# sine2pi/ASR-model

Measured on AMD Instinct MI355X. Metric: audio-sec/sec fwd+bwd on 30s@16kHz LibriSpeech-shaped clips (whole job, all GPUs), higher is better.
Workload: dtype bf16; 1 GPU; tiny (BASELINE configs[1]): log-mel + 4 enc/4 dec d=384 h=6 fwd+bwd, 32 x 30 s clips per GPU, T=256; model=tiny, global_batch=32, seq_len=3001, text_len=256, pitch_frames=3001, parallelism=dp1

## Files before the change

### asr-model_amd/asrx/lib.py

```python
from __future__ import annotations

import ctypes
import os

import torch

_HERE = os.path.dirname(os.path.abspath(__file__))
LIB_PATH = os.environ.get("ASRX_LIB") or os.path.join(_HERE, "libasrx.so")

_i64 = ctypes.c_int64
_i32 = ctypes.c_int
_f32 = ctypes.c_float
_p = ctypes.c_void_p
_u32 = ctypes.c_uint32

SIGNATURES = {
    "asrx_last_error": (ctypes.c_char_p, []),
    "asrx_abi_version": (_i32, []),
    "asrx_noise_hash": (_u32, [_u32, _u32]),
    "asrx_set_noise_epoch": (_i32, [_u32, _p]),
    "asrx_set_gemm_variant": (_i32, [_i32]),
    "asrx_set_attn_variant": (_i32, [_i32]),
    "asrx_set_wgrad_variant": (_i32, [_i32]),
    "asrx_mel_frames": (_i32, [_i64]),
    "asrx_logmel_ws_bytes": (_i64, [_i64, _i64]),
    "asrx_flac_info": (_i32, [_p, _i64, _p, _p, _p, _p, _p]),
    "asrx_flac_decode": (_i32, [_p, _i64, _p, _i64]),
    "asrx_pcm_normalize": (_i32, [_p, _i32, _i64, _i64, _i64, _p, _p, _p, _i64, _i32, _p]),
    "asrx_logmel": (_i32, [_p, _i64, _i64, _i64, _p, _p, _p, _p, _i32, _i64, _p, _p, _i64, _p]),
    "asrx_gemm": (
        _i32,
        [_i32, _p, _i64, _i64, _i32, _i32, _p, _i64, _i64, _i32, _i32, _p, _i64, _i64, _p, _p,
         _i64, _i64, _i64, _i64, _f32, _f32, _i32, _i64, _i64, _i32, _p],
    ),
    "asrx_abby_fwd": (_i32, [_p, _p, _p, _p, _p, _p, _p, _i64, _i64, _i64, _i64, _i64, _u32, _i32, _p]),
    "asrx_abby_fwd_logits": (_i32, [_p, _p, _p, _p, _p, _p, _i64, _i64, _i64, _i64, _i64, _u32, _i32, _p]),
    "asrx_abby_bwd": (_i32, [_p, _p, _p, _p, _p, _p, _p, _p, _p, _p, _i64, _i64, _p]),
    "asrx_attn_fwd": (_i32, [_i32, _p, _p, _p, _p, _p, _p, _p, _p, _p, _i64, _i64, _i64, _i64, _i64, _i32, _f32, _p]),
    "asrx_attn_bwd": (_i32, [_i32, _p, _p, _p, _p, _p, _p, _p, _p, _p, _p, _p, _p, _p, _p, _p, _p, _p, _p,
                             _i64, _i64, _i64, _i64, _i64, _i32, _f32, _p]),
    "asrx_layernorm_fwd": (_i32, [_p, _p, _p, _p, _p, _p, _i64, _i64, _f32, _p]),
    "asrx_layernorm_bwd": (_i32, [_p, _p, _p, _p, _p, _p, _p, _p, _i64, _i64, _p]),
    "asrx_layernorm_bwd_acc": (_i32, [_p, _p, _p, _p, _p, _p, _p, _p, _i64, _i64, _i32, _p]),
    "asrx_small_linear_fwd": (_i32, [_p, _p, _p, _p, _i64, _i64, _i64, _i32, _p]),
    "asrx_small_linear_bwd": (_i32, [_p, _p, _p, _p, _p, _p, _p, _i64, _i64, _i64, _i32, _f32, _p]),
    "asrx_rownorm": (_i32, [_p, _p, _i64, _i64, _p]),
    "asrx_rownorm_bwd": (_i32, [_p, _p, _p, _p, _i64, _i64, _p]),
    "asrx_row_normalize": (_i32, [_p, _p, _p, _i64, _i64, _p]),
    "asrx_row_normalize_bwd": (_i32, [_p, _p, _p, _p, _i64, _i64, _i32, _p]),
    "asrx_softmax_small": (_i32, [_p, _p, _i64, _i64, _p]),
    "asrx_softmax_small_bwd": (_i32, [_p, _p, _p, _i64, _i64, _p]),
    "asrx_zero": (_i32, [_p, _i64, _p]),
    "asrx_rotary_fwd": (_i32, [_p, _p, _p, _p, _i64, _i64, _i64, _i64, _f32, _p]),
    "asrx_rotary_bwd": (_i32, [_p, _p, _p, _p, _p, _p, _i64, _i64, _i64, _i64, _f32, _p]),
    "asrx_abby_bwd2": (_i32, [_p] * 10 + [_i64, _i64, _i32, _p]),
    "asrx_rownorm_bwd2": (_i32, [_p, _p, _p, _p, _i64, _i64, _i32, _p]),
    "asrx_colsum_ld": (_i32, [_p, _i64, _p, _i64, _i64, _p]),
    "asrx_ce_fwd1": (_i32, [_p] * 6 + [_i64, _i64, _p]),
    "asrx_ce_bwd2": (_i32, [_p] * 6 + [_i64, _i64, _p]),
    "asrx_bn_running": (_i32, [_p] * 5 + [_i64, _i64, _i64, _f32, _f32, _p]),
    "asrx_rsqrt_eps": (_i32, [_p, _p, _i64, _f32, _p]),
    "asrx_conv3_weight": (_i32, [_p, _p, _i64, _i64] + [_p] * 6),
    "asrx_conv3_weight_bwd": (_i32, [_p] * 4 + [_i64, _i64] + [_p] * 3),
    "asrx_blend_fwd": (_i32, [_p] * 4 + [_i64, _p]),
    "asrx_blend_bwd": (_i32, [_p] * 7 + [_i64, _p]),
    "asrx_add_segments": (_i32, [_p, _i64, _p, _p, _p, _i64, _p]),
    "asrx_cat3": (_i32, [_p] * 3 + [_i64, _p, _p]),
    "asrx_layernorm_fwd2": (_i32, [_p] * 10 + [_i32, _i64, _i64, _f32, _p]),
    "asrx_vgate_weights": (_i32, [_p] * 7 + [_i64, _i64, _i64, _p]),
    "asrx_msheath_row_fwd": (_i32, [_p] * 6 + [_i64] + [_p] * 14 + [_i64] * 4 + [_f32, _f32, _p, _i64, _i64, _p]),
    "asrx_msheath_row_bwd": (_i32, [_p] * 11 + [_i64] + [_p] * 18 + [_i64] * 4 + [_f32, _p, _i64, _i64, _p]),
    "asrx_msheath_row_bwd2": (_i32, [_i32, _p, _p, _p, _f32, _p] + [_p] * 11 + [_i64] + [_p] * 18 + [_i64] * 4
                              + [_f32, _p, _i64, _i64, _p]),
    "asrx_gemm_wn_rows": (_i32, [_p, _i64, _p, _i64, _p, _i64, _p, _p, _i64, _i64, _i64, _f32, _f32, _i32, _i32, _p,
                                 _p, _p]),
    "asrx_row_tiles_max": (_i64, [_i64]),
    "asrx_wgrad_bf16": (_i32, [_p, _i64, _p, _i64, _p, _i64, _i64, _i64, _i64, _i64, _p]),
    "asrx_pitch_dio": (_i32, [_p, _i64, _i64, _i64] + [ctypes.c_double] * 5 + [_p, _i64, _p, _p, _p, _p, _i64]
                       + [_p] * 4 + [_i64] + [_p] * 4 + [_i64, _p]),
    "asrx_pitch_stonemask": (_i32, [_p, _i64, _i64, _i64, ctypes.c_double, _p, ctypes.c_double, _i64, _p, _p]),
    "asrx_wconv_entry_bytes": (_i64, []),
    "asrx_weights_to_bf16": (_i32, [_p, _i64, _i64, _p]),
    "asrx_row_tiles": (_i32, [_p, _i64, _i64, _i64, _p, _p, _p]),
    "asrx_msheath_ctrl_fwd3": (_i32, [_p, _p, _i64, _p, _p, _p, _p, _p, _i64, _p, _p, _p, _p] + [_i64] * 5 + [_p] * 8),
    "asrx_mem_chunks": (_i64, [_i64]),
    "asrx_seg_colsum_det": (_i32, [_p, _p, _p, _i64, _i64, _i64, _f32, _p]),
    "asrx_msheath_ctrl_bwd3": (_i32, [_p, _p, _p, _p, _p, _p, _i64, _p, _p, _p] + [_i64] * 4 + [_p, _i32] + [_p] * 8),
    "asrx_axpy_row2_colsum": (_i32, [_p] * 6 + [_i64] * 3 + [_p, _i64, _p]),
    "asrx_vgate_fwd": (_i32, [_p, _p, _p, _p, _p, _p, _p, _p, _p, _p, _p, _p, _p, _i64, _i64, _i64, _f32, _p]),
    "asrx_vgate_bwd": (_i32, [_p, _p, _p, _p, _p, _p, _p, _p, _p, _p, _p, _p, _p, _p, _p, _p, _p,
                              _i64, _i64, _i64, _f32, _p]),
    "asrx_tgate_fwd": (_i32, [_p, _p, _p, _i64, _i64, _p]),
    "asrx_tgate_bwd": (_i32, [_p, _p, _p, _p, _p, _i64, _i64, _p]),
    "asrx_axpy_row": (_i32, [_p, _p, _p, _p, _i64, _i64, _p]),
    "asrx_axpy_row_bwd": (_i32, [_p, _p, _p, _p, _p, _i64, _i64, _p]),
    "asrx_axpy_row_bwd2": (_i32, [_p, _p, _p, _p, _p, _p, _i64, _i64, _p]),
    "asrx_jump_select": (_i32, [_p, _p, _p, _p, _p, _p, _p, _p, _i64, _i64, _i64, _p]),
    "asrx_jump_select_bwd": (_i32, [_p, _p, _p, _p, _p, _p, _p, _p, _p, _p, _p, _p, _i64, _i64, _i64, _p]),
    "asrx_seg_colsum": (_i32, [_p, _p, _i64, _i64, _i64, _f32, _i32, _p]),
    "asrx_msheath_ctrl_fwd": (_i32, [_p, _p, _i64, _p, _p, _p, _p, _p, _p, _i64, _i64, _i64, _i64, _i64,
                                     _p, _p, _p, _p, _p, _p, _p, _p]),
    "asrx_msheath_ctrl_bwd": (_i32, [_p, _p, _p, _p, _p, _p, _p, _p, _p, _i64, _i64, _i64, _i64, _p, _p, _p, _p, _p,
                                     _p]),
    "asrx_msheath_rec_bytes": (_i64, []),
    "asrx_msheath_ctrl_fwd2": (_i32, [_p, _p, _i64, _p, _p, _p, _i64, _p, _p, _p, _i64, _i64, _i64, _i64, _i64,
                                      _p, _p, _p, _p, _p, _p, _p, _p]),
    "asrx_msheath_ctrl_bwd2": (_i32, [_p, _p, _p, _p, _p, _p, _i64, _p, _p, _p, _i64, _i64, _i64, _i64, _p, _i32,
                                      _p, _p, _p, _p, _p, _p]),
    "asrx_jump_select4_bwd_acc": (_i32, [_p, _p, _p, _p, _p, _p, _p, _p, _p, _p, _p, _p, _p, _i64, _i64, _i64, _p]),
    "asrx_jump_bwd_part_floats": (_i64, [_i64, _i64, _i64]),
    "asrx_jump_select4_bwd_part": (_i32, [_p] * 11 + [_i64, _i64, _i64, _p]),
    "asrx_msheath_ctrl_bwd4": (_i32, [_p, _i64, _p, _p, _p, _i64, _p, _p, _p, _i64, _i64, _i64, _i64, _p, _i32]
                               + [_p] * 8),
    "asrx_axpy_row2_bwd_acc": (_i32, [_p, _p, _f32, _p, _p, _p, _p, _p, _p, _p, _p, _i64, _i64, _i64, _p]),
    "asrx_jump_select4_bwd_part2": (_i32, [_p] * 11 + [_i64, _i64, _i64, _p]),
    "asrx_jump_select4_bwd_acc2": (_i32, [_p] * 13 + [_i64, _i64, _i64, _p]),
    "asrx_axpy_row2_bwd_acc2": (_i32, [_p, _p, _p, _f32, _p, _p, _p, _p, _p, _p, _p, _p, _i64, _i64, _i64, _p]),
    "asrx_wgrad_split": (_i32, [_p, _i64, _p, _i32, _i64, _p, _i64, _p, _i64, _i64, _i64, _i64, _i64, _i64, _p]),
    "asrx_msheath_dx_final": (_i32, [_p, _p, _p, _p, _i64, _i64, _i64, _p]),
    "asrx_axpy_row2": (_i32, [_p, _p, _p, _p, _p, _i64, _i64, _p]),
    "asrx_axpy_row2_bwd": (_i32, [_p, _p, _p, _p, _p, _p, _p, _i64, _i64, _p]),
    "asrx_jump_select4": (_i32, [_p, _p, _p, _p, _p, _p, _p, _p, _i64, _i64, _i64, _p]),
    "asrx_jump_select4_bwd": (_i32, [_p, _p, _p, _p, _p, _p, _p, _p, _p, _p, _p, _p, _i64, _i64, _i64, _p]),
    "asrx_colsum": (_i32, [_p, _p, _i64, _i64, _p]),
    "asrx_add_rows": (_i32, [_p, _p, _p, _p, _i64, _i64, _i64, _p]),
    "asrx_lincomb": (_i32, [_p, _p, _p, _f32, _f32, _f32, _p, _i64, _p]),
    "asrx_act_fwd": (_i32, [_p, _p, _i64, _i32, _p]),
    "asrx_act_bwd": (_i32, [_p, _p, _p, _i64, _i32, _p]),
    "asrx_glu_fwd": (_i32, [_p, _p, _i64, _i64, _p]),
    "asrx_glu_bwd": (_i32, [_p, _p, _p, _i64, _i64, _p]),
    "asrx_dropout": (_i32, [_p, _p, _i64, _i64, _i64, _i64, _u32, _f32, _p]),
    "asrx_act_dropout_fwd": (_i32, [_p, _p, _p, _i64, _i64, _i64, _i64, _u32, _f32, _i32, _i32, _p]),
    "asrx_act_dropout_bwd": (_i32, [_p, _p, _p, _i64, _i64, _i64, _i64, _u32, _f32, _i32, _i32, _p]),
    "asrx_dwconv_fwd": (_i32, [_p, _p, _p, _p, _i64, _i64, _i64, _i64, _p]),
    "asrx_dwconv_bwd": (_i32, [_p, _p, _p, _p, _p, _p, _i64, _i64, _i64, _i64, _p]),
    "asrx_bn_fwd": (_i32, [_p, _p, _p, _p, _p, _p, _i64, _i64, _i64, _f32, _i32, _p]),
    "asrx_bn_bwd": (_i32, [_p, _p, _p, _p, _p, _p, _p, _p, _p, _p, _i64, _i64, _i64, _p]),
    "asrx_dwconv_pre_bwd": (_i32, [_p, _p, _p, _p, _p, _p, _p, _i64, _i64, _i64, _i64, _i32, _p]),
    "asrx_bn_silu_fwd": (_i32, [_p, _p, _p, _p, _p, _p, _i64, _i64, _i64, _f32, _i32, _p]),
    "asrx_bn_silu_bwd": (_i32, [_p, _p, _p, _p, _p, _p, _p, _p, _p, _p, _p, _i64, _i64, _i64, _p]),
    "asrx_stem1_fwd": (_i32, [_p, _p, _p, _p, _i64, _i64, _i64, _p]),
    "asrx_stem1_bwd": (_i32, [_p, _p, _p, _p, _i64, _i64, _i64, _p]),
    "asrx_embed_fwd": (_i32, [_p, _p, _p, _i64, _i64, _p]),
    "asrx_embed_bwd": (_i32, [_p, _p, _p, _i64, _i64, _p]),
    "asrx_ce_fwd": (_i32, [_p, _p, _p, _p, _i64, _i64, _p]),
    "asrx_ce_bwd": (_i32, [_p, _p, _p, _p, _p, _i64, _i64, _p]),
    "asrx_policy_noise": (_i32, [_p, _i64, _i64, _i64, _u32, _p]),
    "asrx_weight_to_bf16": (_i32, [_p, _p, _i64, _i64, _i64, _i32, _p]),
    "asrx_gemm_wn_router": (_i32, [_p, _i64, _p, _i64, _p, _p, _p, _i64, _p, _i64, _i64, _i64, _p]),
    "asrx_gemm_wn": (_i32, [_p, _i64, _i32, _i64, _i64, _p, _i64, _p, _i64, _p, _p, _i64, _i64, _i64, _f32, _f32,
                            _i32, _i32, _p]),
    "asrx_gemm_wn_ex": (_i32, [_p, _i32, _i64, _i32, _i64, _i64, _p, _i64, _p, _i32, _i64, _p, _p, _i64, _i64, _i64,
                               _f32, _f32, _i32, _i32, _p, _p, _p]),
    "asrx_wgrad_bf16_ex": (_i32, [_p, _i64, _p, _i32, _i64, _p, _i64, _i64, _i64, _i64, _i64, _p]),
    "asrx_abby_fwd2": (_i32, [_p, _p, _p, _p, _p, _i32, _p, _p, _i64, _i64, _i64, _i64, _i64, _u32, _i32, _p, _p, _p,
                              _p]),
    "asrx_gemm_wn_gact": (_i32, [_p, _i32, _i64, _p, _i64, _p, _p, _i64, _p, _i64, _p, _i64, _i64, _i64, _i32, _i32,
                                 _p]),
    "asrx_rotary_table": (_i32, [_p, _p, _i64, _i64, _p]),
    "asrx_rotary_fwd2": (_i32, [_p, _p, _p, _p, _p, _i64, _i64, _i64, _i64, _f32, _p]),
    "asrx_rotary_bwd2": (_i32, [_p, _p, _p, _p, _p, _p, _p, _i64, _i64, _i64, _i64, _f32, _p]),
    "asrx_abby_fwd3": (_i32, [_p, _p, _p, _p, _p, _p, _i32, _p, _p, _i64, _i64, _i64, _i64, _i64, _u32, _i32, _p, _p,
                               _p, _p, _p]),
    "asrx_abby_fwd_logits2": (_i32, [_p, _p, _p, _p, _i32, _p, _p, _i64, _i64, _i64, _i64, _i64, _u32, _i32, _p, _p,
                                     _p, _p]),
    "asrx_attn_fwd2": (_i32, [_i32, _i32, _p, _p, _p, _p, _p, _p, _p, _p, _p, _i64, _i64, _i64, _i64, _i64, _i32, _f32,
                              _p]),
    "asrx_attn_bwd2": (_i32, [_i32, _i32, _p, _p, _p, _p, _p, _p, _p, _p, _p, _p, _p, _p, _p, _p, _p, _p, _p, _p,
                              _i64, _i64, _i64, _i64, _i64, _i32, _f32, _p]),
    "asrx_small_linear_fwd2": (_i32, [_p, _i32, _p, _p, _p, _i64, _i64, _i64, _i32, _p]),
    "asrx_small_linear_bwd2": (_i32, [_p, _p, _p, _i32, _p, _p, _p, _p, _i64, _i64, _i64, _i32, _f32, _p]),
    "asrx_tgate_fwd2": (_i32, [_p, _p, _p, _i32, _i64, _i64, _p]),
    "asrx_msheath_row_fwd2": (_i32, [_p] * 6 + [_i64] + [_p] * 7 + [_i32] + [_p] * 7 + [_i64] * 4
                                    + [_f32, _f32, _p, _i64, _i64, _p]),
    "asrx_msheath_row_fwd3": (_i32, [_p] * 6 + [_i64] + [_p] * 16 + [_i64] * 4 + [_f32, _f32, _p, _i64, _i64, _p]),
# ... 125 lines not shown
```

### asr-model_amd/csrc/attn_mf.hip

```cpp
#include "common.h"

namespace asrx {

struct AttnStridesMF {
  int64_t b, l, h;
};

typedef short v4i16 __attribute__((ext_vector_type(4)));
typedef __attribute__((address_space(3))) v4i16 lds_v4i16;

namespace amf {

constexpr int QB = 256;
constexpr int KT = 64;
constexpr int NTHR = 512;
constexpr int HALF = KT * 64;
constexpr float LOG2E = 1.4426950408889634f;
constexpr float LN2 = 0.6931471805599453f;

__device__ __forceinline__ int kswz(int key) { return (key >> 1) & 7; }
__device__ __forceinline__ int vswz(int key) { return ((key >> 1) & 1) << 2; }

__device__ __forceinline__ unsigned pack2(float a, float b) {
  typedef __attribute__((ext_vector_type(2))) float f2;
// ... 546 lines not shown
          const int ql = 32 * qb2 + 8 * (2 * s2 + e4) + 4 * hi;
          const float4 lo = *reinterpret_cast<const float4*>(&LD[buf][ql]);
          const float4 hi4 = *reinterpret_cast<const float4*>(&LD[buf][ql + 2]);
          const float l2v[4] = {lo.x, lo.z, hi4.x, hi4.z}, dlv[4] = {lo.y, lo.w, hi4.y, hi4.w};
#pragma unroll
          for (int e = 0; e < 4; e += 2) {
            typedef __attribute__((ext_vector_type(2))) float f2;
            const int r = 8 * s2 + 4 * e4 + e;
            const f2 a = __builtin_elementwise_fma((f2){sacc[r], sacc[r + 1]}, (f2){c, c}, (f2){-l2v[e], -l2v[e + 1]});
            f2 p = {__builtin_amdgcn_exp2f(a.x), __builtin_amdgcn_exp2f(a.y)};
            if (need_mask) {
              p.x = kq > ql + e ? 0.f : p.x;
              p.y = kq > ql + e + 1 ? 0.f : p.y;
            }
            const f2 ds = p * ((f2){pacc[r], pacc[r + 1]} - (f2){dlv[e], dlv[e + 1]});
            pv[4 * e4 + e] = p.x;
            pv[4 * e4 + e + 1] = p.y;
            dsv[4 * e4 + e] = ds.x;
            dsv[4 * e4 + e + 1] = ds.y;
          }
        }
        const bf16x8 pb = pack8(pv), sb = pack8(dsv);
#pragma unroll
        for (int d = 0; d < HD / 32; ++d) {
          dvacc[d] = __builtin_amdgcn_mfma_f32_32x32x16_bf16(tr_frag(Dt[buf] + (d >> 1) * HALF, lane, qb2, s2, d & 1),
                                                             pb, dvacc[d], 0, 0, 0);
          dkacc[d] = __builtin_amdgcn_mfma_f32_32x32x16_bf16(tr_frag(Qt[buf] + (d >> 1) * HALF, lane, qb2, s2, d & 1),
                                                             sb, dkacc[d], 0, 0, 0);
        }
      }
    }
    if (t + 1 < ntiles) stage_st(buf ^ 1);
    __syncthreads();
  }

  if (key < Lk) {
    store_rowT<HD>(dk + b * sdk.b + h * sdk.h + key * sdk.l, dkacc, scale, hi);
    store_rowT<HD>(dv + b * sdv.b + h * sdv.h + key * sdv.l, dvacc, 1.f, hi);
  }
}

template <int HD, typename TI = float, typename TD = float>
__global__ __launch_bounds__(BwdCfg<HD>::NT, 1) void attn_bwd_dq_mf_kernel(
    const TI* __restrict__ q, const TI* __restrict__ k, const TI* __restrict__ v,
    const TD* __restrict__ dO, const float* __restrict__ lse, const float* __restrict__ delta,
    float* __restrict__ dq, AttnStridesMF sq, AttnStridesMF sk, AttnStridesMF sv, AttnStridesMF sd,
    AttnStridesMF sdq, int64_t H, int64_t Lq, int64_t Lk, int causal, float scale) {
  typedef BwdCfg<HD> C;
  constexpr int NH = HD / 64;
  __shared__ __attribute__((aligned(16))) unsigned short Kr[2][NH * HALF], Kt2[2][NH * HALF], Vr[2][NH * HALF];

  const int64_t nqb = (Lq + 32 * C::NW - 1) / (32 * C::NW), L = xcd_logical(blockIdx.x, gridDim.x);
  const int b = (int)(L / (nqb * H)), h = (int)((L / nqb) % H);
  const int64_t q0 = (L % nqb) * (32 * C::NW);
  const int tid = threadIdx.x, lane = tid & 63, wid = __builtin_amdgcn_readfirstlane(tid >> 6);
  const int j = lane & 31, hi = lane >> 5;
  const int64_t qi = q0 + wid * 32 + j;
  const TI* kbp = k + b * sk.b + h * sk.h;
  const TI* vbp = v + b * sv.b + h * sv.h;
  const float c = scale * LOG2E;

  bf16x8 qf[HD / 16], gf[HD / 16];
  row_frags<HD>(q + b * sq.b + h * sq.h, sq.l, qi, Lq, hi, qf);
  row_frags<HD>(dO + b * sd.b + h * sd.h, sd.l, qi, Lq, hi, gf);
  const float l2 = qi < Lq ? lse[((int64_t)b * H + h) * Lq + qi] * LOG2E : 0.f;
  const float dl = qi < Lq ? delta[((int64_t)b * H + h) * Lq + qi] : 0.f;

  int64_t kend = Lk;
  if (causal) kend = min(Lk, q0 + 32 * C::NW);
  const int ntiles = (int)((kend + KT - 1) / KT);
  const int skey = tid >> 3, sc = tid & 7;

  Row8<TI> ka[C::RI][NH], va[C::RI][NH];
  auto stage_ld = [&](int64_t k0) {
#pragma unroll
    for (int i = 0; i < C::RI; ++i)
#pragma unroll
      for (int hf = 0; hf < NH; ++hf) {
        stage_load(kbp, sk, k0 + skey + i * (C::NT / 8), Lk, hf, sc, ka[i][hf]);
        stage_load(vbp, sv, k0 + skey + i * (C::NT / 8), Lk, hf, sc, va[i][hf]);
      }
  };
  auto stage_st = [&](int buf) {
#pragma unroll
    for (int i = 0; i < C::RI; ++i)
#pragma unroll
      for (int hf = 0; hf < NH; ++hf) {
        const int row = skey + i * (C::NT / 8);
        stage_store(Kr[buf] + hf * HALF, row, sc ^ kswz(row), ka[i][hf]);
        stage_store(Kt2[buf] + hf * HALF, row, sc ^ vswz(row), ka[i][hf]);
        stage_store(Vr[buf] + hf * HALF, row, sc ^ kswz(row), va[i][hf]);
      }
  };
  stage_ld(0);
  stage_st(0);
  __syncthreads();

  f32x16 dqacc[HD / 32];
#pragma unroll
  for (int d = 0; d < HD / 32; ++d)
#pragma unroll
    for (int r = 0; r < 16; ++r) dqacc[d][r] = 0.f;

  for (int t = 0; t < ntiles; ++t) {
    const int buf = t & 1;
    const int64_t k0 = (int64_t)t * KT;
    if (t + 1 < ntiles) stage_ld(k0 + KT);
    f32x16 sacc[2], pacc[2];
#pragma unroll
    for (int kb2 = 0; kb2 < 2; ++kb2) {
#pragma unroll
      for (int r = 0; r < 16; ++r) {
        sacc[kb2][r] = 0.f;
        pacc[kb2][r] = 0.f;
      }
      dot_rows<HD>(sacc[kb2], Kr[buf], 32 * kb2 + j, hi, qf);
      dot_rows<HD>(pacc[kb2], Vr[buf], 32 * kb2 + j, hi, gf);
    }
    const bool need_mask =
        __builtin_amdgcn_readfirstlane((int)((k0 + KT > Lk) || (causal && k0 + KT - 1 > q0 + wid * 32))) != 0;
    const int lim = need_mask ? (int)min(min(Lk - k0, (int64_t)KT), causal ? qi - k0 + 1 : (int64_t)KT) : KT;
    bf16x8 sb[2][2];
#pragma unroll
    for (int kb2 = 0; kb2 < 2; ++kb2)
#pragma unroll
      for (int s2 = 0; s2 < 2; ++s2) {
        float dsv[8];
#pragma unroll
        for (int e = 0; e < 8; e += 2) {
          typedef __attribute__((ext_vector_type(2))) float f2;
          const int r = 8 * s2 + e;
          const f2 a = __builtin_elementwise_fma((f2){sacc[kb2][r], sacc[kb2][r + 1]}, (f2){c, c}, (f2){-l2, -l2});
          f2 p = {__builtin_amdgcn_exp2f(a.x), __builtin_amdgcn_exp2f(a.y)};
          if (need_mask) {
            p.x = (32 * kb2 + (r & 3) + 8 * (r >> 2) + 4 * hi) >= lim ? 0.f : p.x;
            p.y = (32 * kb2 + ((r + 1) & 3) + 8 * ((r + 1) >> 2) + 4 * hi) >= lim ? 0.f : p.y;
          }
          const f2 ds = p * ((f2){pacc[kb2][r], pacc[kb2][r + 1]} - (f2){dl, dl});
          dsv[e] = ds.x;
          dsv[e + 1] = ds.y;
        }
        sb[kb2][s2] = pack8(dsv);
      }
#pragma unroll
    for (int kb2 = 0; kb2 < 2; ++kb2)
#pragma unroll
      for (int s2 = 0; s2 < 2; ++s2)
#pragma unroll
        for (int d = 0; d < HD / 32; ++d)
          dqacc[d] = __builtin_amdgcn_mfma_f32_32x32x16_bf16(tr_frag(Kt2[buf] + (d >> 1) * HALF, lane, kb2, s2, d & 1),
                                                             sb[kb2][s2], dqacc[d], 0, 0, 0);
    if (t + 1 < ntiles) stage_st(buf ^ 1);
    __syncthreads();
  }

  if (qi < Lq) store_rowT<HD>(dq + b * sdq.b + h * sdq.h + qi * sdq.l, dqacc, scale, hi);
}

}

static int g_attn_fwd_variant = 1;

template <int HD, typename TI, typename TO>
static void attn_fwd_mf_t(const void* q, AttnStridesMF Sq, const void* k, AttnStridesMF Sk, const void* v,
                          AttnStridesMF Sv, void* o, AttnStridesMF So, float* lse, int64_t B, int64_t H, int64_t Lq,
                          int64_t Lk, int causal, float scale, hipStream_t stream) {
  const TI *qq = (const TI*)q, *kk = (const TI*)k, *vv = (const TI*)v;
  TO* oo = (TO*)o;
  dim3 g((unsigned)((Lq + amf::QB - 1) / amf::QB), (unsigned)H, (unsigned)B);
  if (HD == 64 && g_attn_fwd_variant == 1) {
    if (g.x > 1)
      amf::attn_fwd_sp_kernel<true, TI, TO><<<dim3((unsigned)((int64_t)g.x * g.y * g.z)), amf::NTHR, 0, stream>>>(
          qq, kk, vv, oo, lse, Sq, Sk, Sv, So, H, Lq, Lk, causal, scale);
    else
      amf::attn_fwd_sp_kernel<false, TI, TO><<<g, amf::NTHR, 0, stream>>>(qq, kk, vv, oo, lse, Sq, Sk, Sv, So, H, Lq,
                                                                          Lk, causal, scale);
  } else if (HD == 64 && g.x > 1)
    amf::attn_fwd_mf_kernel<HD, 1, true, false, TI, TO><<<dim3((unsigned)((int64_t)g.x * g.y * g.z)), amf::NTHR, 0,
                                                          stream>>>(qq, kk, vv, oo, lse, Sq, Sk, Sv, So, H, Lq, Lk,
                                                                    causal, scale);
  else
    amf::attn_fwd_mf_kernel<HD, 1, false, false, TI, TO><<<g, amf::NTHR, 0, stream>>>(qq, kk, vv, oo, lse, Sq, Sk, Sv,
                                                                                     So, H, Lq, Lk, causal, scale);
}

int attn_fwd_mf(int io, const void* q, const int64_t* sq, const void* k, const int64_t* sk, const void* v,
                const int64_t* sv, void* o, const int64_t* so, float* lse, int64_t B, int64_t H, int64_t Lq,
                int64_t Lk, int64_t hd, int causal, float scale, hipStream_t stream) {
  AttnStridesMF Sq{sq[0], sq[1], sq[2]}, Sk{sk[0], sk[1], sk[2]}, Sv{sv[0], sv[1], sv[2]}, So{so[0], so[1], so[2]};
#define ASRX_AF(HDV, TI, TO) attn_fwd_mf_t<HDV, TI, TO>(q, Sq, k, Sk, v, Sv, o, So, lse, B, H, Lq, Lk, causal, scale, stream)
  if (hd == 64) {
    switch (io & 3) {
      case 0: ASRX_AF(64, float, float); break;
      case 1: ASRX_AF(64, amf::bf16s, float); break;
      case 2: ASRX_AF(64, float, amf::bf16s); break;
      default: ASRX_AF(64, amf::bf16s, amf::bf16s); break;
    }
  } else {
    switch (io & 3) {
      case 0: ASRX_AF(128, float, float); break;
      case 1: ASRX_AF(128, amf::bf16s, float); break;
      case 2: ASRX_AF(128, float, amf::bf16s); break;
      default: ASRX_AF(128, amf::bf16s, amf::bf16s); break;
    }
  }
#undef ASRX_AF
  return 0;
}

template <int HD, typename TI, typename TD>
static void attn_bwd_mf_t(const void* q, AttnStridesMF Sq, const void* k, AttnStridesMF Sk, const void* v,
                          AttnStridesMF Sv, const void* dO, AttnStridesMF Sd, const float* lse, const float* delta,
                          float* dq, AttnStridesMF Sdq, float* dk, AttnStridesMF Sdk, float* dv, AttnStridesMF Sdv,
                          int64_t B, int64_t H, int64_t Lq, int64_t Lk, int causal, float scale, hipStream_t stream) {
  typedef amf::BwdCfg<HD> C;
  const TI *qq = (const TI*)q, *kk = (const TI*)k, *vv = (const TI*)v;
  const TD* gg = (const TD*)dO;
  const int64_t rows_per_wg = 32 * C::NW;
  dim3 gk((unsigned)(((Lk + rows_per_wg - 1) / rows_per_wg) * H * B));
  amf::attn_bwd_dkdv_mf_kernel<HD, TI, TD><<<gk, C::NT, 0, stream>>>(qq, kk, vv, gg, lse, delta, dk, dv, Sq, Sk, Sv, Sd,
                                                                     Sdk, Sdv, H, Lq, Lk, causal, scale);
  dim3 gq((unsigned)(((Lq + rows_per_wg - 1) / rows_per_wg) * H * B));
  amf::attn_bwd_dq_mf_kernel<HD, TI, TD><<<gq, C::NT, 0, stream>>>(qq, kk, vv, gg, lse, delta, dq, Sq, Sk, Sv, Sd, Sdq,
                                                                   H, Lq, Lk, causal, scale);
}

int attn_bwd_mf(int io, const void* q, const int64_t* sq, const void* k, const int64_t* sk, const void* v,
                const int64_t* sv, const void* dO, const int64_t* sd, const float* lse, const float* delta,
                float* dq, const int64_t* sdq, float* dk, const int64_t* sdk, float* dv, const int64_t* sdv,
                int64_t B, int64_t H, int64_t Lq, int64_t Lk, int64_t hd, int causal, float scale,
                hipStream_t stream) {
  AttnStridesMF Sq{sq[0], sq[1], sq[2]}, Sk{sk[0], sk[1], sk[2]}, Sv{sv[0], sv[1], sv[2]}, Sd{sd[0], sd[1], sd[2]};
  AttnStridesMF Sdq{sdq[0], sdq[1], sdq[2]}, Sdk{sdk[0], sdk[1], sdk[2]}, Sdv{sdv[0], sdv[1], sdv[2]};
#define ASRX_AB(HDV, TI, TD)                                                                                       \
  attn_bwd_mf_t<HDV, TI, TD>(q, Sq, k, Sk, v, Sv, dO, Sd, lse, delta, dq, Sdq, dk, Sdk, dv, Sdv, B, H, Lq, Lk, causal, \
                             scale, stream)
  const int sel = (io & 1) | ((io >> 1) & 2);
  if (hd == 64) {
    switch (sel) {
      case 0: ASRX_AB(64, float, float); break;
      case 1: ASRX_AB(64, amf::bf16s, float); break;
      case 2: ASRX_AB(64, float, amf::bf16s); break;
      default: ASRX_AB(64, amf::bf16s, amf::bf16s); break;
    }
  } else {
    switch (sel) {
      case 0: ASRX_AB(128, float, float); break;
      case 1: ASRX_AB(128, amf::bf16s, float); break;
      case 2: ASRX_AB(128, float, amf::bf16s); break;
      default: ASRX_AB(128, amf::bf16s, amf::bf16s); break;
    }
  }
#undef ASRX_AB
  return 0;
}

}

extern "C" int asrx_set_attn_variant(int v) {
  const int old = asrx::g_attn_fwd_variant;
  asrx::g_attn_fwd_variant = v;
  return old;
}
```

### include/asrx.h

```cpp
#ifndef ASRX_H
#define ASRX_H
#include <stdint.h>

#ifdef __cplusplus
extern "C" {
#endif

typedef void* asrx_stream_t;

const char* asrx_last_error(void);
int asrx_abi_version(void);
uint32_t asrx_noise_hash(uint32_t key, uint32_t idx);
int asrx_set_noise_epoch(uint32_t epoch, asrx_stream_t stream);
int asrx_set_gemm_variant(int variant);
int asrx_set_attn_variant(int variant);
int asrx_set_wgrad_variant(int variant);

int asrx_mel_frames(int64_t n_samples);
int64_t asrx_logmel_ws_bytes(int64_t B, int64_t N);
int asrx_logmel(const float* wav, int64_t B, int64_t N, int64_t ld_wav, const float* consts,
                const float* fbw, const int* fbs, float* out, int layout, int64_t ld_out,
                void* ws, float* pool, int64_t T_pool, asrx_stream_t stream);
int asrx_wave_pool(const float* wav, int64_t B, int64_t N, int64_t ld_wav, int64_t T, float* out,
                   asrx_stream_t stream);
int asrx_logmel_ragged(const float* wav, int64_t B, int64_t Nmax, int64_t ld_wav, const void* clips,
                       const float* consts, const float* fbw, const int* fbs, float* out, int layout,
                       int64_t ld_out, int64_t Fmax, void* ws, float* pool, int64_t Tmax,
                       asrx_stream_t stream);
int asrx_wave_pool_ragged(const float* wav, int64_t B, int64_t Nmax, int64_t ld_wav, const void* clips,
                          float* out, int64_t Tmax, asrx_stream_t stream);

int asrx_flac_info(const uint8_t* buf, int64_t n, int64_t* frames, int* channels, int* rate, int* bits,
                   uint8_t* md5);
int asrx_flac_decode(const uint8_t* buf, int64_t n, int32_t* out, int64_t cap);
int asrx_pcm_normalize(const void* pcm, int is_float, int64_t B, int64_t C, int64_t ld, const int64_t* lengths,
                       const float* scale, float* out, int64_t ld_out, int normalize, asrx_stream_t stream);

int asrx_gemm(int prec, const float* A, int64_t lda, int64_t sA, int a_kc, int conv_a,
              const float* B, int64_t ldb, int64_t sB, int b_kc, int conv_b, float* C, int64_t ldc,
              int64_t sC, const float* bias, float* Z, int64_t M, int64_t N, int64_t K,
              int64_t batch, float alpha, float beta, int act, int64_t conv_F, int64_t conv_C,
              int splitk, asrx_stream_t stream);


int asrx_weight_to_bf16(const float* src, unsigned short* dst, int64_t rows, int64_t cols, int64_t ld, int trans,
                        asrx_stream_t stream);
int64_t asrx_wconv_entry_bytes(void);
int asrx_weights_to_bf16(const void* tab, int64_t n, int64_t max_elems, asrx_stream_t stream);
int asrx_gemm_wn_router(const float* A, int64_t lda, const unsigned short* W1, int64_t ldw, const float* b1,
                        const float* W2, float* hpre, int64_t ldc, float* logits, int64_t M, int64_t N, int64_t K,
                        asrx_stream_t stream);
int asrx_gemm_wn(const float* A, int64_t lda, int conv, int64_t convF, int64_t convC, const unsigned short* W,
                 int64_t ldw, float* C, int64_t ldc, const float* bias, float* Z, int64_t M, int64_t N, int64_t K,
                 float alpha, float beta, int act, int nj, asrx_stream_t stream);
int asrx_wgrad_bf16(const float* A, int64_t lda, const float* B, int64_t ldb, float* C, int64_t ldc, int64_t M,
                    int64_t N, int64_t R, int64_t splitk, asrx_stream_t stream);
int asrx_gemm_wn_rows(const float* A, int64_t lda, const unsigned short* W, int64_t ldw, float* C, int64_t ldc,
                      const float* bias, float* Z, int64_t M, int64_t N, int64_t K, float alpha, float beta, int act,
                      int nj, const int* mtiles, const int* n_mtiles, asrx_stream_t stream);
int asrx_gemm_wn_ex(const void* A, int a_bf16, int64_t lda, int conv, int64_t convF, int64_t convC,
                    const unsigned short* W, int64_t ldw, void* C, int c_bf16, int64_t ldc, const float* bias,
                    float* Z, int64_t M, int64_t N, int64_t K, float alpha, float beta, int act, int nj,
                    const int* mtiles, const int* n_mtiles, asrx_stream_t stream);
int asrx_wgrad_bf16_ex(const float* A, int64_t lda, const void* B, int b_bf16, int64_t ldb, float* C, int64_t ldc,
                       int64_t M, int64_t N, int64_t R, int64_t splitk, asrx_stream_t stream);
int64_t asrx_row_tiles_max(int64_t M);
int asrx_row_tiles(const float* next_i, int64_t layer, int64_t L, int64_t M, int* mtiles, int* n_mtiles,
                   asrx_stream_t stream);

int asrx_abby_record_cond(unsigned char* buf);
int asrx_abby_fwd(const float* x, const float* hpre, const float* W2, const float* b2, float* out, float* ys,
                  int* idx, int64_t rows, int64_t d, int64_t L, int64_t H, int64_t sid_base, uint32_t key,
                  int use_noise, asrx_stream_t stream);
int asrx_abby_fwd_res(const float* x, const float* hpre, const float* W2, const float* logits, const float* b2,
                      const float* res, float* out, float* ys, int* idx, int64_t rows, int64_t d, int64_t L, int64_t H,
                      int64_t sid_base, uint32_t key, int use_noise, asrx_stream_t stream);
int asrx_abby_fwd_logits(const float* x, const float* logits, const float* b2, float* out, float* ys, int* idx,
                         int64_t rows, int64_t d, int64_t L, int64_t H, int64_t sid_base, uint32_t key,
                         int use_noise, asrx_stream_t stream);
int asrx_abby_fwd2(const float* x, const float* hpre, const float* W2, const float* b2, void* out, int out_bf16,
                   float* ys, int* idx, int64_t rows, int64_t d, int64_t L, int64_t H, int64_t sid_base, uint32_t key,
                   int use_noise, const float* tw, const float* tb, float* tc, asrx_stream_t stream);
int asrx_abby_fwd_logits2(const float* x, const float* logits, const float* b2, void* out, int out_bf16, float* ys,
                          int* idx, int64_t rows, int64_t d, int64_t L, int64_t H, int64_t sid_base, uint32_t key,
                          int use_noise, const float* tw, const float* tb, float* tc, asrx_stream_t stream);
int asrx_abby_fwd3(const float* x, const float* hpre, const float* W2, const float* logits, const float* b2,
                   void* out, int out_bf16, float* ys, int* idx, int64_t rows, int64_t d, int64_t L, int64_t H,
                   int64_t sid_base, uint32_t key, int use_noise, const float* tw, const float* tb, float* tc,
                   float* nrm, asrx_stream_t stream);
int asrx_abby_bwd(const float* dout, const float* x, const float* hpre, const float* W2, const float* ys,
                  const int* idx, float* dx, float* dhpre, float* dW2, float* db2, int64_t rows, int64_t d,
                  asrx_stream_t stream);
int asrx_abby_bwd2(const float* dout, const float* x, const float* hpre, const float* W2, const float* ys,
                   const int* idx, float* dx, float* dhpre, float* dW2, float* db2, int64_t rows, int64_t d, int acc,
                   asrx_stream_t stream);

int asrx_attn_fwd(int prec, const float* q, const int64_t* sq, const float* k, const int64_t* sk, const float* v,
                  const int64_t* sv, float* o, const int64_t* so, float* lse, int64_t B, int64_t H, int64_t Lq,
                  int64_t Lk, int64_t hd, int causal, float scale, asrx_stream_t stream);
int asrx_attn_fwd2(int prec, int io, const void* q, const int64_t* sq, const void* k, const int64_t* sk,
                   const void* v, const int64_t* sv, void* o, const int64_t* so, float* lse, int64_t B, int64_t H,
                   int64_t Lq, int64_t Lk, int64_t hd, int causal, float scale, asrx_stream_t stream);
int asrx_attn_bwd2(int prec, int io, const void* q, const int64_t* sq, const void* k, const int64_t* sk,
                   const void* v, const int64_t* sv, const void* o, const int64_t* so, const void* dO,
                   const int64_t* sd, const float* lse, float* delta_ws, float* dq, const int64_t* sdq, float* dk,
                   const int64_t* sdk, float* dv, const int64_t* sdv, int64_t B, int64_t H, int64_t Lq, int64_t Lk,
                   int64_t hd, int causal, float scale, asrx_stream_t stream);
int asrx_attn_bwd(int prec, const float* q, const int64_t* sq, const float* k, const int64_t* sk, const float* v,
                  const int64_t* sv, const float* o, const int64_t* so, const float* dO, const int64_t* sd,
                  const float* lse, float* delta_ws, float* dq, const int64_t* sdq, float* dk, const int64_t* sdk,
                  float* dv, const int64_t* sdv, int64_t B, int64_t H, int64_t Lq, int64_t Lk, int64_t hd,
                  int causal, float scale, asrx_stream_t stream);

int asrx_layernorm_fwd(const float* x, const float* w, const float* b, float* y, float* mean, float* rstd,
                       int64_t rows, int64_t d, float eps, asrx_stream_t stream);
int asrx_layernorm_bwd(const float* dy, const float* x, const float* w, const float* mean, const float* rstd,
                       float* dx, float* dw, float* db, int64_t rows, int64_t d, asrx_stream_t stream);
int asrx_layernorm_bwd_acc(const float* dy, const float* x, const float* w, const float* mean, const float* rstd,
                           float* dx, float* dw, float* db, int64_t rows, int64_t d, int acc, asrx_stream_t stream);

int asrx_layernorm_fwd2(const float* x, const float* w, const float* b, float* y, float* mean, float* rstd,
                        float* nrm, const float* gw, const float* gb, float* gout, int gate_on_x, int64_t rows,
                        int64_t d, float eps, asrx_stream_t stream);
int asrx_layernorm_fwd3(const float* x, const float* w, const float* b, void* y, int y_bf16, float* mean, float* rstd,
                        float* nrm, const float* gw, const float* gb, float* gout, int gate_on_x, int64_t rows,
                        int64_t d, float eps, asrx_stream_t stream);

int asrx_small_linear_fwd(const float* x, const float* W, const float* b, float* y, int64_t rows, int64_t K,
                          int64_t N, int act, asrx_stream_t stream);
int asrx_small_linear_bwd(const float* dy, const float* y, const float* x, const float* W, float* dx, float* dW,
                          float* db, int64_t rows, int64_t K, int64_t N, int act, float beta,
                          asrx_stream_t stream);
int asrx_small_linear_fwd2(const void* x, int x_bf16, const float* W, const float* b, float* y, int64_t rows,
                           int64_t K, int64_t N, int act, asrx_stream_t stream);
int asrx_small_linear_bwd2(const float* dy, const float* y, const void* x, int x_bf16, const float* W, float* dx,
                           float* dW, float* db, int64_t rows, int64_t K, int64_t N, int act, float beta,
                           asrx_stream_t stream);

int asrx_rownorm(const float* x, float* n, int64_t rows, int64_t d, asrx_stream_t stream);
int asrx_rownorm_bwd(const float* dn, const float* x, const float* n, float* dx, int64_t rows, int64_t d,
                     asrx_stream_t stream);
int asrx_rownorm_bwd2(const float* dn, const float* x, const float* n, float* dx, int64_t rows, int64_t d, int acc,
                      asrx_stream_t stream);
int asrx_row_normalize(const float* x, float* y, float* n, int64_t rows, int64_t d, asrx_stream_t stream);
int asrx_row_normalize_bwd(const float* dy, const float* y, const float* n, float* dx, int64_t rows, int64_t d,
                           int acc, asrx_stream_t stream);
int asrx_softmax_small(const float* x, float* y, int64_t rows, int64_t N, asrx_stream_t stream);
int asrx_softmax_small_bwd(const float* g, const float* y, float* dx, int64_t rows, int64_t N, asrx_stream_t stream);
int asrx_zero(void* p, int64_t bytes, asrx_stream_t stream);

int asrx_rotary_fwd(const float* x, const float* m, const float* f, float* y, int64_t BL, int64_t L, int64_t D,
                    int64_t hd, float scale, asrx_stream_t stream);
int asrx_rotary_bwd(const float* g, const float* x, const float* m, const float* f, float* dx, float* dm,
                    int64_t BL, int64_t L, int64_t D, int64_t hd, float scale, asrx_stream_t stream);
int asrx_rotary_table(const float* f, float* tab, int64_t L, int64_t hd, asrx_stream_t stream);
int asrx_rotary_fwd2(const float* x, const float* m, const float* f, const float* tab, float* y, int64_t BL, int64_t L,
                     int64_t D, int64_t hd, float scale, asrx_stream_t stream);
int asrx_rotary_bwd2(const float* g, const float* x, const float* m, const float* f, const float* tab, float* dx,
                     float* dm, int64_t BL, int64_t L, int64_t D, int64_t hd, float scale, asrx_stream_t stream);

int asrx_vgate_fwd(const float* S, const float* nx, const float* mval, const float* h, const float* w2,
                   const float* b2, const float* cw, const float* cb, const float* tx, float* ion, float* xval,
                   float* kv, float* m2, int64_t rows, int64_t M, int64_t Dh, float inv_sqrt_d,
                   asrx_stream_t stream);
int asrx_vgate_bwd(const float* dion, const float* S, const float* nx, const float* mval, const float* h,
                   const float* w2, const float* cw, const float* kv, const float* m2, float* dS, float* dnx,
                   float* dh, float* dmval, float* dw2, float* db2, float* dcw, float* dcb, int64_t rows, int64_t M,
                   int64_t Dh, float inv_sqrt_d, asrx_stream_t stream);
// ... 293 lines not shown
```

Measured before the change: 5547 audio-sec/sec.

## Add specialized hd=64 attention backward kernels with mask-free tiles and precomputed LDS offsets

Adds new dK/dV and dQ backward kernels for head dim 64 and makes them the default through a new variant switch. They precompute swizzled LDS fragment offsets once per lane, split each tile into masked and unmasked compile-time paths chosen per wave, and prefetch lse/delta pairs into LDS alongside the Q/dO tiles. The aim is to cut per-tile address arithmetic and mask selects in the inner loop. The cost is extra duplicated code and extra LDS for the lse/delta buffer, and the opaque() barrier may constrain instruction scheduling.

```diff
diff --git a/asr-model_amd/asrx/lib.py b/asr-model_amd/asrx/lib.py
--- a/asr-model_amd/asrx/lib.py
+++ b/asr-model_amd/asrx/lib.py
@@ -21,6 +21,7 @@
     "asrx_set_noise_epoch": (_i32, [_u32, _p]),
     "asrx_set_gemm_variant": (_i32, [_i32]),
     "asrx_set_attn_variant": (_i32, [_i32]),
+    "asrx_set_attn_bwd_variant": (_i32, [_i32]),
     "asrx_set_wgrad_variant": (_i32, [_i32]),
     "asrx_mel_frames": (_i32, [_i64]),
     "asrx_logmel_ws_bytes": (_i64, [_i64, _i64]),
diff --git a/asr-model_amd/csrc/attn_mf.hip b/asr-model_amd/csrc/attn_mf.hip
--- a/asr-model_amd/csrc/attn_mf.hip
+++ b/asr-model_amd/csrc/attn_mf.hip
@@ -722,6 +722,279 @@
                                                              sb[kb2][s2], dqacc[d], 0, 0, 0);
     if (t + 1 < ntiles) stage_st(buf ^ 1);
     __syncthreads();
+  }
+
+  if (qi < Lq) store_rowT<HD>(dq + b * sdq.b + h * sdq.h + qi * sdq.l, dqacc, scale, hi);
+}
+
+
+__device__ __forceinline__ float opaque(float x) {
+  asm("" : "+v"(x));
+  return x;
+}
+
+template <bool B>
+struct BoolC {
+  static constexpr bool value = B;
+};
+
+struct FragOffs {
+  int row[4], tr[2];
+};
+__device__ __forceinline__ FragOffs frag_offs(int lane) {
+  const int j = lane & 31, hi = lane >> 5;
+  const int g = lane >> 4, gi = lane & 15, trow = 4 * (g >> 1) + (gi >> 2), tcol = 4 * (gi & 3);
+  FragOffs o;
+#pragma unroll
+  for (int s = 0; s < 4; ++s) o.row[s] = j * 64 + 8 * ((2 * s + hi) ^ kswz(j));
+#pragma unroll
+  for (int dd = 0; dd < 2; ++dd) {
+    const int col = 32 * dd + 16 * (g & 1) + tcol;
+    o.tr[dd] = trow * 64 + 8 * ((col >> 3) ^ vswz(trow)) + (col & 7);
+  }
+  return o;
+}
+__device__ __forceinline__ void dot_rows_o(f32x16& acc, const unsigned short* X, int half, const FragOffs& o,
+                                           const bf16x8 (&f)[4]) {
+#pragma unroll
+  for (int s = 0; s < 4; ++s)
+    acc = __builtin_amdgcn_mfma_f32_32x32x16_bf16(*reinterpret_cast<const bf16x8*>(X + half * (32 * 64) + o.row[s]),
+                                                  f[s], acc, 0, 0, 0);
+}
+__device__ __forceinline__ bf16x8 tr_frag_o(const unsigned short* X, const FragOffs& o, int kb2, int s2, int dd) {
+  const unsigned short* p = X + (32 * kb2 + 16 * s2) * 64 + o.tr[dd];
+  const v4i16 t1 = __builtin_amdgcn_ds_read_tr16_b64_v4i16((lds_v4i16*)p);
+  const v4i16 t2 = __builtin_amdgcn_ds_read_tr16_b64_v4i16((lds_v4i16*)(p + 8 * 64));
+  typedef short v8i16 __attribute__((ext_vector_type(8)));
+  const v8i16 a8 = {t1[0], t1[1], t1[2], t1[3], t2[0], t2[1], t2[2], t2[3]};
+  return __builtin_bit_cast(bf16x8, a8);
+}
+
+template <typename TI, typename TD>
+__global__ __launch_bounds__(NTHR, 1) void attn_bwd_dkdv_v1_kernel(
+    const TI* __restrict__ q, const TI* __restrict__ k, const TI* __restrict__ v,
+    const TD* __restrict__ dO, const float* __restrict__ lse, const float* __restrict__ delta,
+    float* __restrict__ dk, float* __restrict__ dv, AttnStridesMF sq, AttnStridesMF sk, AttnStridesMF sv,
+    AttnStridesMF sd, AttnStridesMF sdk, AttnStridesMF sdv, int64_t H, int64_t Lq, int64_t Lk, int causal,
+    float scale) {
+  constexpr int HD = 64;
+  typedef BwdCfg<HD> C;
+  __shared__ __attribute__((aligned(16))) unsigned short Qr[2][HALF], Qt[2][HALF];
+  __shared__ __attribute__((aligned(16))) unsigned short Dr[2][HALF], Dt[2][HALF];
+  __shared__ __attribute__((aligned(16))) float2 LD[2][BQT];
+
+  const int64_t nkb = (Lk + 32 * C::NW - 1) / (32 * C::NW), L = xcd_logical(blockIdx.x, gridDim.x);
+  const int b = (int)(L / (nkb * H)), h = (int)((L / nkb) % H);
+  const int64_t k0 = (L % nkb) * (32 * C::NW);
+  const int tid = threadIdx.x, lane = tid & 63, wid = __builtin_amdgcn_readfirstlane(tid >> 6);
+  const int j = lane & 31, hi = lane >> 5;
+  const int64_t key = k0 + wid * 32 + j;
+  const TI* qb = q + b * sq.b + h * sq.h;
+  const TD* gb = dO + b * sd.b + h * sd.h;
+  const float* lb = lse + ((int64_t)b * H + h) * Lq;
+  const float* db = delta + ((int64_t)b * H + h) * Lq;
+  const float c = scale * LOG2E;
+  const FragOffs fo = frag_offs(lane);
+
+  bf16x8 kf[HD / 16], vf[HD / 16];
+  row_frags<HD>(k + b * sk.b + h * sk.h, sk.l, key, Lk, hi, kf);
+  row_frags<HD>(v + b * sv.b + h * sv.h, sv.l, key, Lk, hi, vf);
+
+  const int64_t qt0 = causal ? k0 / BQT : 0;
+  const int ntiles = (int)((Lq + BQT - 1) / BQT - qt0);
+  const int srow = tid >> 3, sc = tid & 7;
+  Row8<TI> qa;
+  Row8<TD> ga;
+  float2 ld = make_float2(0.f, 0.f);
+  auto stage_ld = [&](int t) {
+    const int64_t q0 = (qt0 + t) * BQT;
+    stage_load(qb, sq, q0 + srow, Lq, 0, sc, qa);
+    stage_load(gb, sd, q0 + srow, Lq, 0, sc, ga);
+    if (tid < BQT) {
+      const int64_t qi = q0 + tid;
+      ld = qi < Lq ? make_float2(lb[qi] * LOG2E, db[qi]) : make_float2(INFINITY, 0.f);
+    }
+  };
+  auto stage_st = [&](int buf) {
+    stage_store(Qr[buf], srow, sc ^ kswz(srow), qa);
+    stage_store(Qt[buf], srow, sc ^ vswz(srow), qa);
+    stage_store(Dr[buf], srow, sc ^ kswz(srow), ga);
+    stage_store(Dt[buf], srow, sc ^ vswz(srow), ga);
+    if (tid < BQT) LD[buf][tid] = ld;
+  };
+
+  f32x16 dvacc[HD / 32], dkacc[HD / 32];
+#pragma unroll
+  for (int d = 0; d < HD / 32; ++d)
+#pragma unroll
+    for (int r = 0; r < 16; ++r) {
+      dvacc[d][r] = 0.f;
+      dkacc[d][r] = 0.f;
+    }
+  if (ntiles > 0) {
+    stage_ld(0);
+    stage_st(0);
+  }
+  __syncthreads();
+
+  auto tile = [&](auto mk, int buf, int kq) {
+    constexpr bool MASK = decltype(mk)::value;
+#pragma unroll
+    for (int qb2 = 0; qb2 < 2; ++qb2) {
+      f32x16 sacc, pacc;
+#pragma unroll
+      for (int r = 0; r < 16; ++r) {
+        sacc[r] = 0.f;
+        pacc[r] = 0.f;
+      }
+      dot_rows_o(sacc, Qr[buf], qb2, fo, kf);
+      dot_rows_o(pacc, Dr[buf], qb2, fo, vf);
+#pragma unroll
+      for (int s2 = 0; s2 < 2; ++s2) {
+        float pv[8], dsv[8];
+#pragma unroll
+        for (int e4 = 0; e4 < 2; ++e4) {
+          const int ql = 32 * qb2 + 8 * (2 * s2 + e4) + 4 * hi;
+          const float4 lo = *reinterpret_cast<const float4*>(&LD[buf][ql]);
+          const float4 hi4 = *reinterpret_cast<const float4*>(&LD[buf][ql + 2]);
+          const float l2v[4] = {lo.x, lo.z, hi4.x, hi4.z}, dlv[4] = {lo.y, lo.w, hi4.y, hi4.w};
+#pragma unroll
+          for (int e = 0; e < 4; ++e) {
+            const int r = 8 * s2 + 4 * e4 + e;
+            float p = __builtin_amdgcn_exp2f(__builtin_fmaf(sacc[r], c, -l2v[e]));
+            if constexpr (MASK) p = kq > ql + e ? 0.f : p;
+            pv[4 * e4 + e] = p;
+            dsv[4 * e4 + e] = opaque(p * (pacc[r] - dlv[e]));
+          }
+        }
+        const bf16x8 pb = pack8(pv), sb = pack8(dsv);
+#pragma unroll
+        for (int d = 0; d < HD / 32; ++d) {
+          dvacc[d] = __builtin_amdgcn_mfma_f32_32x32x16_bf16(tr_frag_o(Dt[buf], fo, qb2, s2, d), pb, dvacc[d], 0, 0, 0);
+          dkacc[d] = __builtin_amdgcn_mfma_f32_32x32x16_bf16(tr_frag_o(Qt[buf], fo, qb2, s2, d), sb, dkacc[d], 0, 0, 0);
+        }
+      }
+    }
+  };
+  auto step = [&](int t, int buf) {
+    const int64_t q0 = (qt0 + t) * BQT;
+    if (t + 1 < ntiles) stage_ld(t + 1);
+    if (__builtin_amdgcn_readfirstlane((int)(causal && q0 < k0 + wid * 32 + 32)) != 0)
+      tile(BoolC<true>{}, buf, (int)(key - q0));
+    else
+      tile(BoolC<false>{}, buf, 0);
+    if (t + 1 < ntiles) stage_st(buf ^ 1);
+    __syncthreads();
+  };
+  for (int t = 0; t < ntiles; t += 2) {
+    step(t, 0);
+    if (t + 1 < ntiles) step(t + 1, 1);
+  }
+
+  const int ln = __builtin_amdgcn_mbcnt_hi(~0u, __builtin_amdgcn_mbcnt_lo(~0u, 0u));
+  const int64_t key_st = k0 + wid * 32 + (ln & 31);
+  if (key_st < Lk) {
+    store_rowT<HD>(dk + b * sdk.b + h * sdk.h + key_st * sdk.l, dkacc, scale, ln >> 5);
+    store_rowT<HD>(dv + b * sdv.b + h * sdv.h + key_st * sdv.l, dvacc, 1.f, ln >> 5);
+  }
+}
+
+template <typename TI, typename TD>
+__global__ __launch_bounds__(NTHR, 1) void attn_bwd_dq_v1_kernel(
+    const TI* __restrict__ q, const TI* __restrict__ k, const TI* __restrict__ v,
+    const TD* __restrict__ dO, const float* __restrict__ lse, const float* __restrict__ delta,
+    float* __restrict__ dq, AttnStridesMF sq, AttnStridesMF sk, AttnStridesMF sv, AttnStridesMF sd,
+    AttnStridesMF sdq, int64_t H, int64_t Lq, int64_t Lk, int causal, float scale) {
+  constexpr int HD = 64;
+  typedef BwdCfg<HD> C;
+  __shared__ __attribute__((aligned(16))) unsigned short Kr[2][HALF], Kt2[2][HALF], Vr[2][HALF];
+
+  const int64_t nqb = (Lq + 32 * C::NW - 1) / (32 * C::NW), L = xcd_logical(blockIdx.x, gridDim.x);
+  const int b = (int)(L / (nqb * H)), h = (int)((L / nqb) % H);
+  const int64_t q0 = (L % nqb) * (32 * C::NW);
+  const int tid = threadIdx.x, lane = tid & 63, wid = __builtin_amdgcn_readfirstlane(tid >> 6);
+  const int j = lane & 31, hi = lane >> 5;
+  const int64_t qi = q0 + wid * 32 + j;
+  const TI* kbp = k + b * sk.b + h * sk.h;
+  const TI* vbp = v + b * sv.b + h * sv.h;
+  const float c = scale * LOG2E;
+  const FragOffs fo = frag_offs(lane);
+
+  bf16x8 qf[HD / 16], gf[HD / 16];
+  row_frags<HD>(q + b * sq.b + h * sq.h, sq.l, qi, Lq, hi, qf);
+  row_frags<HD>(dO + b * sd.b + h * sd.h, sd.l, qi, Lq, hi, gf);
+  const float l2 = qi < Lq ? lse[((int64_t)b * H + h) * Lq + qi] * LOG2E : 0.f;
+  const float dl = qi < Lq ? delta[((int64_t)b * H + h) * Lq + qi] : 0.f;
+
+  int64_t kend = Lk;
+  if (causal) kend = min(Lk, q0 + 32 * C::NW);
+  const int ntiles = (int)((kend + KT - 1) / KT);
+  const int skey = tid >> 3, sc = tid & 7;
+
+  Row8<TI> ka, va;
+  auto stage_ld = [&](int64_t k0) {
+    stage_load(kbp, sk, k0 + skey, Lk, 0, sc, ka);
+    stage_load(vbp, sv, k0 + skey, Lk, 0, sc, va);
+  };
+  auto stage_st = [&](int buf) {
+    stage_store(Kr[buf], skey, sc ^ kswz(skey), ka);
+    stage_store(Kt2[buf], skey, sc ^ vswz(skey), ka);
+    stage_store(Vr[buf], skey, sc ^ kswz(skey), va);
+  };
+  stage_ld(0);
+  stage_st(0);
+  __syncthreads();
+
+  f32x16 dqacc[HD / 32];
+#pragma unroll
+  for (int d = 0; d < HD / 32; ++d)
+#pragma unroll
+    for (int r = 0; r < 16; ++r) dqacc[d][r] = 0.f;
+
+  auto tile = [&](auto mk, int buf, int lim) {
+    constexpr bool MASK = decltype(mk)::value;
+    f32x16 sacc[2], pacc[2];
+#pragma unroll
+    for (int kb2 = 0; kb2 < 2; ++kb2) {
+#pragma unroll
+      for (int r = 0; r < 16; ++r) {
+        sacc[kb2][r] = 0.f;
+        pacc[kb2][r] = 0.f;
+      }
+      dot_rows_o(sacc[kb2], Kr[buf], kb2, fo, qf);
+      dot_rows_o(pacc[kb2], Vr[buf], kb2, fo, gf);
+    }
+#pragma unroll
+    for (int kb2 = 0; kb2 < 2; ++kb2)
+#pragma unroll
+      for (int s2 = 0; s2 < 2; ++s2) {
+        float dsv[8];
+#pragma unroll
+        for (int e = 0; e < 8; ++e) {
+          const int r = 8 * s2 + e;
+          float p = __builtin_amdgcn_exp2f(__builtin_fmaf(sacc[kb2][r], c, -l2));
+          if constexpr (MASK) p = (32 * kb2 + (r & 3) + 8 * (r >> 2) + 4 * hi) >= lim ? 0.f : p;
+          dsv[e] = opaque(p * (pacc[kb2][r] - dl));
+        }
+        const bf16x8 sb = pack8(dsv);
+#pragma unroll
+        for (int d = 0; d < HD / 32; ++d)
+          dqacc[d] = __builtin_amdgcn_mfma_f32_32x32x16_bf16(tr_frag_o(Kt2[buf], fo, kb2, s2, d), sb, dqacc[d], 0, 0, 0);
+      }
+  };
+  auto step = [&](int t, int buf) {
+    const int64_t k0 = (int64_t)t * KT;
+    if (t + 1 < ntiles) stage_ld(k0 + KT);
+    if (__builtin_amdgcn_readfirstlane((int)((k0 + KT > Lk) || (causal && k0 + KT - 1 > q0 + wid * 32))) != 0)
+      tile(BoolC<true>{}, buf, (int)min(min(Lk - k0, (int64_t)KT), causal ? qi - k0 + 1 : (int64_t)KT));
+    else
+      tile(BoolC<false>{}, buf, KT);
+    if (t + 1 < ntiles) stage_st(buf ^ 1);
+    __syncthreads();
+  };
+  for (int t = 0; t < ntiles; t += 2) {
+    step(t, 0);
+    if (t + 1 < ntiles) step(t + 1, 1);
   }
 
   if (qi < Lq) store_rowT<HD>(dq + b * sdq.b + h * sdq.h + qi * sdq.l, dqacc, scale, hi);
@@ -778,6 +1051,8 @@
   return 0;
 }
 
+static int g_attn_bwd_variant = 1;
+
 template <int HD, typename TI, typename TD>
 static void attn_bwd_mf_t(const void* q, AttnStridesMF Sq, const void* k, AttnStridesMF Sk, const void* v,
                           AttnStridesMF Sv, const void* dO, AttnStridesMF Sd, const float* lse, const float* delta,
@@ -788,9 +1063,18 @@
   const TD* gg = (const TD*)dO;
   const int64_t rows_per_wg = 32 * C::NW;
   dim3 gk((unsigned)(((Lk + rows_per_wg - 1) / rows_per_wg) * H * B));
+  dim3 gq((unsigned)(((Lq + rows_per_wg - 1) / rows_per_wg) * H * B));
+  if constexpr (HD == 64) {
+    if (g_attn_bwd_variant == 1) {
+      amf::attn_bwd_dkdv_v1_kernel<TI, TD><<<gk, C::NT, 0, stream>>>(qq, kk, vv, gg, lse, delta, dk, dv, Sq, Sk, Sv, Sd,
+                                                                     Sdk, Sdv, H, Lq, Lk, causal, scale);
+      amf::attn_bwd_dq_v1_kernel<TI, TD><<<gq, C::NT, 0, stream>>>(qq, kk, vv, gg, lse, delta, dq, Sq, Sk, Sv, Sd, Sdq, H,
+                                                                   Lq, Lk, causal, scale);
+      return;
+    }
+  }
   amf::attn_bwd_dkdv_mf_kernel<HD, TI, TD><<<gk, C::NT, 0, stream>>>(qq, kk, vv, gg, lse, delta, dk, dv, Sq, Sk, Sv, Sd,
                                                                      Sdk, Sdv, H, Lq, Lk, causal, scale);
-  dim3 gq((unsigned)(((Lq + rows_per_wg - 1) / rows_per_wg) * H * B));
   amf::attn_bwd_dq_mf_kernel<HD, TI, TD><<<gq, C::NT, 0, stream>>>(qq, kk, vv, gg, lse, delta, dq, Sq, Sk, Sv, Sd, Sdq,
                                                                    H, Lq, Lk, causal, scale);
 }
@@ -832,3 +1116,9 @@
   asrx::g_attn_fwd_variant = v;
   return old;
 }
+
+extern "C" int asrx_set_attn_bwd_variant(int v) {
+  const int old = asrx::g_attn_bwd_variant;
+  asrx::g_attn_bwd_variant = v;
+  return old;
+}
diff --git a/include/asrx.h b/include/asrx.h
--- a/include/asrx.h
+++ b/include/asrx.h
@@ -14,6 +14,7 @@
 int asrx_set_noise_epoch(uint32_t epoch, asrx_stream_t stream);
 int asrx_set_gemm_variant(int variant);
 int asrx_set_attn_variant(int variant);
+int asrx_set_attn_bwd_variant(int variant);
 int asrx_set_wgrad_variant(int variant);
 
 int asrx_mel_frames(int64_t n_samples);
```

New measurement: 5576 audio-sec/sec, median of 6. About the same (+0.5%).
